# arkworks-rs/marlin

Measured on NVIDIA H100. Metric: prover_constraints_per_sec, higher is better.
Workload: dtype u32-limb modular integers (Fr 255-bit, Fq 381-bit)

## Files before the change

marlin_b200/csrc/msm.cuh:

```cuda
#pragma once
#include "common.cuh"
#include "curve.cuh"
#include "msm_layout.hpp"

namespace b2m {

constexpr uint32_t MSM_BKT_MASK = (1u << MSM_BKT_BITS) - 1;
constexpr uint32_t MSM_NO_DIGIT = 0xffffffffu;
constexpr int MSM_MAX_AFFINE_LEVELS = 6;

template <class Fr, class Fq>
struct MsmJob {
  const Fr* scalars;
  bool mont;
  size_t n;
  size_t base_off;
  const Fr* scalars2;
  size_t n2;
  size_t extra_base;
  const XYZZ<Fq>* extra;
  int n_extra;
  XYZZ<Fq>* out_xyzz;
  Affine<Fq>* out_affine;
  size_t scalar_stride = 1;
};

template <class Fr, class Fq>
struct Msm {
  Ctx* ctx;
  size_t n_srs = 0;
  size_t n_srs_global = 0;
  int tab_rank = 0, tab_world = 1;
  size_t n_extra = 0;
  size_t stride = 0;
  int c = 0, W = 0;
  int T = 0, m = 1;
  size_t max_pairs = 0;
  int affine_levels = Fq::N > 8 ? 3 : 0;
  int affine_ctas_upper = 22;
  int affine_ctas = 4;
  size_t affine_min_refs = MSM_AFFINE_MIN_REFS;
  int affine_map = 1;
  int affine_T = 64;
  int affine_T_upper = 32;
  int acc_ctas_per_sm = 3;
  DBuf<Affine<Fq>> tables;

  static int pick_window(size_t n);
  Msm(Ctx& cx, const Affine<Fq>* powers, size_t n, const Affine<Fq>* host_extra, size_t n_extra_bases, int window_bits,
      bool powers_on_device = false, int n_tables = 0, size_t max_pairs = 0);

  void run(const Fr* scalars, bool mont, size_t n, size_t base_off, const XYZZ<Fq>* extra, int n_extra, XYZZ<Fq>* out_xyzz,
           Affine<Fq>* out_affine);
  void run_batch(const MsmJob<Fr, Fq>* jobs, int nj);
  void run_pass(const MsmJob<Fr, Fq>* jobs, int nj);
  void run_host(size_t base_off, const uint64_t* scalars, size_t n, uint64_t* out_xy, int* out_is_inf);
  void read_power(size_t i, uint64_t* out_xy);
  static void g1_to_bytes(Ctx& cx, const Affine<Fq>* dev_pts, const uint64_t* host_pts, size_t n, uint8_t* out);
  static void g1_from_bytes(Ctx& cx, const uint8_t* bytes, size_t n, uint64_t* out_xy);
  static void g1_powers_host(Ctx& cx, const uint64_t* g_xy, const uint64_t* beta, size_t n, uint64_t* out);
  static void fixed_base_host(Ctx& cx, const uint64_t* g_xy, const uint64_t* scalars, const uint64_t* beta, size_t first, size_t n, uint64_t* out);
};

}
```

marlin_b200/csrc/msm_affine.cuh:

```cuda
#pragma once
#include "curve.cuh"
#ifdef __CUDACC__
#include "devmem.cuh"
#else
struct uint2 {
  uint32_t x, y;
};
struct uint4 {
  uint32_t x, y, z, w;
};
#endif

namespace b2m {

constexpr uint32_t AFF_BKT_BITS = 24;

template <class Fq>
struct AffLevel {
  const Affine<Fq>* tables;
  size_t table_stride;
  const uint2* sorted;
  const Affine<Fq>* in;
  const uint32_t* off_in;
  const uint32_t* off_out;
  uint32_t B;
  Affine<Fq>* out;
  uint2* out_refs;
  Fq* pref;
  uint4* meta;
  uint32_t T, nthreads;
  uint32_t lane_step;
  Fq* inv;
};

struct AffMap {
  uint32_t o0, step, cnt;
};
template <class Fq>
B2M_HD AffMap aff_map(const AffLevel<Fq>& A, uint32_t t, uint32_t total) {
  AffMap m;
  m.step = A.lane_step;
  uint64_t o0;
  if (A.lane_step == 1) {
    o0 = (uint64_t)t * A.T;
  } else {
    o0 = (uint64_t)(t / A.lane_step) * A.lane_step * A.T + (t % A.lane_step);
  }
  if (o0 >= total) {
    m.o0 = 0;
    m.cnt = 0;
    return m;
  }
  m.o0 = (uint32_t)o0;
  const uint32_t left = (total - m.o0 + m.step - 1) / m.step;
  m.cnt = left < A.T ? left : A.T;
  return m;
}

#if defined(__CUDA_ARCH__)
#define B2M_AFF_LDG(p) ldg_words(p)
#define B2M_AFF_LD(p) ld_words(p)
#define B2M_AFF_ST(p, v) st_words(p, v)
#define B2M_AFF_LDG32(p) __ldg(p)
#else
#define B2M_AFF_LDG(p) (*(p))
#define B2M_AFF_LD(p) (*(p))
#define B2M_AFF_ST(p, v) (*(p) = (v))
#define B2M_AFF_LDG32(p) (*(p))
#endif

B2M_HD uint32_t aff_bucket_of(const uint32_t* off, uint32_t n, uint32_t v) {
  uint32_t lo = 0, hi = n;
  while (hi - lo > 1) {
    uint32_t mid = (lo + hi) >> 1;
    if (B2M_AFF_LDG32(off + mid) <= v) lo = mid; else hi = mid;
  }
  return lo;
}

template <class Fq, bool L0>
B2M_HD void aff_plan_thread(const AffLevel<Fq>& A, uint32_t t) {
  const uint32_t total = B2M_AFF_LDG32(A.off_out + A.B);
  const AffMap mp = aff_map(A, t, total);
  if (!mp.cnt) return;
  uint32_t b = aff_bucket_of(A.off_out, A.B, mp.o0);
  uint32_t b_start = B2M_AFF_LDG32(A.off_out + b), b_end = B2M_AFF_LDG32(A.off_out + b + 1);
  for (uint32_t k = 0; k < mp.cnt; k++) {
    const uint32_t o = mp.o0 + k * mp.step;
    if (o >= b_end) {
      int steps = 0;
      do {
        b++;
        b_end = B2M_AFF_LDG32(A.off_out + b + 1);
      } while (o >= b_end && ++steps < 8);
      if (o >= b_end) {
        b = aff_bucket_of(A.off_out, A.B, o);
        b_end = B2M_AFF_LDG32(A.off_out + b + 1);
      }
      b_start = B2M_AFF_LDG32(A.off_out + b);
    }
    const uint32_t in_start = B2M_AFF_LDG32(A.off_in + b), in_end = B2M_AFF_LDG32(A.off_in + b + 1);
    const uint32_t i0 = in_start + 2u * (o - b_start);
    const bool pair = i0 + 1u < in_end;
    uint4 m;
    if (L0) {
      const uint2 r0 = B2M_AFF_LDG32(A.sorted + i0);
      m.x = (uint32_t)((size_t)(r0.y >> AFF_BKT_BITS) * A.table_stride + (r0.x & 0x7fffffffu)) | (r0.x & 0x80000000u);
      m.y = m.x;
      if (pair) {
        const uint2 r1 = B2M_AFF_LDG32(A.sorted + i0 + 1u);
        m.y = (uint32_t)((size_t)(r1.y >> AFF_BKT_BITS) * A.table_stride + (r1.x & 0x7fffffffu)) | (r1.x & 0x80000000u);
      }
    } else {
      m.x = i0;
      m.y = pair ? i0 + 1u : i0;
    }
    m.z = b;
    m.w = pair ? 1u : 0u;
    A.meta[(size_t)k * A.nthreads + t] = m;
  }
}

template <class Fq>
B2M_HD Fq aff_ldx(const Affine<Fq>* base, uint32_t ref) {
  return B2M_AFF_LDG(&base[ref & 0x7fffffffu].x);
}
template <class Fq>
B2M_HD Affine<Fq> aff_ld(const Affine<Fq>* base, uint32_t ref) {
  const Affine<Fq>* p = base + (ref & 0x7fffffffu);
  Affine<Fq> r;
  r.x = B2M_AFF_LDG(&p->x);
  r.y = B2M_AFF_LDG(&p->y);
  return r;
}
template <class Fq>
B2M_HD Affine<Fq> aff_signed(Affine<Fq> p, uint32_t ref) {
  if (ref >> 31) p.y = p.y.neg();
  return p;
}

enum AffKind : uint32_t { AFF_COPY_P = 0, AFF_COPY_Q = 1, AFF_INF = 2, AFF_ADD = 3, AFF_DBL = 4 };

template <class Fq>
B2M_HD AffKind aff_classify(const Affine<Fq>& P, const Affine<Fq>& Q, Fq* den) {
  if (P.is_inf()) return AFF_COPY_Q;
  if (Q.is_inf()) return AFF_COPY_P;
  if (P.x == Q.x) {
    if (P.y == Q.y && !P.y.is_zero()) {
      *den = P.y.dbl();
      return AFF_DBL;
    }
    return AFF_INF;
  }
  *den = Q.x - P.x;
  return AFF_ADD;
}

template <class Fq, bool PF>
B2M_HD void aff_level_thread(const AffLevel<Fq>& A, const Affine<Fq>* base, uint32_t t) {
  const uint32_t total = B2M_AFF_LDG32(A.off_out + A.B);
// ... 280 lines not shown
```

marlin_b200/csrc/msm_impl.cuh:

```cuda
#pragma once
#include "msm.cuh"
#include "devmem.cuh"
#include "scan.cuh"
#include "msm_affine.cuh"
#include "comm.cuh"

namespace b2m {

template <class Fq>
__device__ __forceinline__ Affine<Fq> ld_affine(const Affine<Fq>* p) {
  Affine<Fq> r;
  const uint4* q = reinterpret_cast<const uint4*>(p);
  uint32_t* d = reinterpret_cast<uint32_t*>(&r);
#pragma unroll
  for (int i = 0; i < 2 * Fq::N / 4; i++) {
    uint4 v = __ldg(q + i);
    d[4 * i] = v.x; d[4 * i + 1] = v.y; d[4 * i + 2] = v.z; d[4 * i + 3] = v.w;
  }
  return r;
}
template <class Fq> __device__ __noinline__ void g1_add(XYZZ<Fq>& a, const XYZZ<Fq>& b) { a.add(b); }
template <class Fq> __device__ __noinline__ void g1_add_mixed(XYZZ<Fq>& a, const Affine<Fq>& b) { a.add_mixed(b); }
template <class Fq> __device__ __noinline__ void g1_dbl(XYZZ<Fq>& a) { a = a.dbl(); }
template <class Fq> __device__ __noinline__ Fq fq_inverse(const Fq& a) { return a.inverse_fast(); }
// ... 67 lines not shown
      carry = 0;
      out = v ? (set_off + v - 1) : MSM_NO_DIGIT;
    }
    digits[(size_t)w * nt + i] = out;
    if (out != MSM_NO_DIGIT) atomicAdd(hist + (out & 0x7fffffffu), 1u);
  }
}


static __global__ void msm_scatter_kernel(const uint32_t* digits, size_t n, size_t nt, size_t base_off, size_t idx2, int W, int m,
                                          uint32_t* cursor, uint2* sorted) {
  size_t i = blockIdx.x * (size_t)blockDim.x + threadIdx.x;
  if (i >= nt) return;
  uint32_t abs_idx = (uint32_t)(i < n ? base_off + i : idx2 + (i - n));
  for (int w = 0; w < W; w++) {
    uint32_t d = digits[(size_t)w * nt + i];
    if (d == MSM_NO_DIGIT) continue;
    uint32_t bkt = d & 0x7fffffffu;
    uint32_t pos = atomicAdd(cursor + bkt, 1u);
    sorted[pos] = make_uint2(abs_idx | (d & 0x80000000u), bkt | ((uint32_t)(w / m) << MSM_BKT_BITS));
  }
}

constexpr int MSM_Q = 64;
constexpr int MSM_Q_MIN = 32;
template <class Fq>
__global__ void __launch_bounds__(128)
msm_accumulate_kernel(const Affine<Fq>* __restrict__ tables, size_t table_stride, const uint32_t* __restrict__ offsets,
                      const uint32_t* __restrict__ ends, const uint2* __restrict__ sorted, const uint32_t* __restrict__ total_refs_p,
                      const uint32_t q, XYZZ<Fq>* __restrict__ buckets, XYZZ<Fq>* __restrict__ part_pt,
                      uint32_t* __restrict__ part_bkt) {
  const uint32_t total = *total_refs_p;
  const uint32_t t = blockIdx.x * blockDim.x + threadIdx.x;
  const uint64_t start64 = (uint64_t)t * q;
  uint32_t head_b = MSM_NO_DIGIT, tail_b = MSM_NO_DIGIT;
  if (start64 < total) {
    const uint32_t start = (uint32_t)start64;
    const uint32_t end = (total - start > q) ? start + q : total;
    uint2 rb = __ldg(sorted + start);
    uint32_t ref = rb.x;
    uint32_t cur_b = rb.y & MSM_BKT_MASK;
    uint32_t seg_start = start;
    Affine<Fq> p = ld_affine(tables + (size_t)(rb.y >> MSM_BKT_BITS) * table_stride + (ref & 0x7fffffffu));
    XYZZ<Fq> acc = XYZZ<Fq>::inf();
    for (uint32_t e = start; e < end; e++) {
      Affine<Fq> cur = p;
      const bool neg = ref >> 31;
      uint32_t next_b = cur_b;
      if (e + 1 < end) {
        rb = __ldg(sorted + e + 1);
        ref = rb.x;
        next_b = rb.y & MSM_BKT_MASK;
        p = ld_affine(tables + (size_t)(rb.y >> MSM_BKT_BITS) * table_stride + (ref & 0x7fffffffu));
      }
      acc.add_mixed(cur, neg);
      if (e + 1 == end || next_b != cur_b) {
        const bool whole = (seg_start == offsets[cur_b]) && (e + 1 == ends[cur_b]);
        if (whole) {
          st_words(buckets + cur_b, acc);
        } else if (seg_start == start && head_b == MSM_NO_DIGIT) {
          st_words(part_pt + 2 * (size_t)t, acc);
          head_b = cur_b;
        } else {
          st_words(part_pt + 2 * (size_t)t + 1, acc);
          tail_b = cur_b;
        }
        acc = XYZZ<Fq>::inf();
        seg_start = e + 1;
        cur_b = next_b;
      }
    }
  }
  part_bkt[2 * (size_t)t] = head_b;
  part_bkt[2 * (size_t)t + 1] = tail_b;
}
static __global__ void msm_level_counts_kernel(const uint32_t* off_in, uint32_t B, uint32_t* cnt) {
  uint32_t b = blockIdx.x * blockDim.x + threadIdx.x;
  if (b > B) return;
  cnt[b] = b < B ? (off_in[b + 1] - off_in[b] + 1u) / 2u : 0u;
}
template <class Fq, bool L0>
__global__ void __launch_bounds__(256) msm_affine_plan_kernel(const AffLevel<Fq> A) {
  const uint32_t t = blockIdx.x * blockDim.x + threadIdx.x;
  if (t < A.nthreads) aff_plan_thread<Fq, L0>(A, t);
}
template <class Fq, int MINB, bool PF>
__global__ void __launch_bounds__(128, MINB) msm_affine_level_kernel(const AffLevel<Fq> A, const Affine<Fq>* __restrict__ base) {
  const uint32_t t = blockIdx.x * blockDim.x + threadIdx.x;
  if (t < A.nthreads) aff_level_thread<Fq, PF>(A, base, t);
}

template <class Fq, int MINB, int PHASE, bool PIPE = true>
__global__ void __launch_bounds__(128, MINB) msm_affine_level_sp_kernel(const AffLevel<Fq> A, const Affine<Fq>* __restrict__ base) {
  const uint32_t t = blockIdx.x * blockDim.x + threadIdx.x;
  if (t < A.nthreads) aff_level_thread_sp<Fq, PHASE, PIPE>(A, base, t);
}

template <class Fq>
__device__ __forceinline__ Fq shfl_fq(const Fq& a, int src_lane) {
  Fq r;
#pragma unroll
  for (int i = 0; i < Fq::N; i++) r.l[i] = __shfl_sync(0xffffffffu, a.l[i], src_lane);
  return r;
}
template <class Fq>
__global__ void __launch_bounds__(128) fq_batch_inverse_kernel(Fq* v, size_t n) {
  constexpr int G = 4;
  const size_t t = blockIdx.x * (size_t)blockDim.x + threadIdx.x;
  const int lane = threadIdx.x & 31;
  const size_t i0 = t * G;
  Fq e[G], pre[G];
  Fq run = Fq::one();
#pragma unroll
  for (int k = 0; k < G; k++) {
    e[k] = i0 + k < n ? ld_words(v + i0 + k) : Fq::one();
    pre[k] = run;
    run = run * e[k];
  }
  Fq pin = run, sin = run;
#pragma unroll
  for (int d = 1; d < 32; d <<= 1) {
    const Fq up = shfl_fq(pin, lane - d < 0 ? lane : lane - d);
    const Fq dn = shfl_fq(sin, lane + d > 31 ? lane : lane + d);
    if (lane >= d) pin = pin * up;
    if (lane + d <= 31) sin = sin * dn;
  }
  Fq tinv = Fq::one();
  if (lane == 31) tinv = fq_inverse(pin);
  tinv = shfl_fq(tinv, 31);
  Fq before = shfl_fq(pin, lane == 0 ? 0 : lane - 1), after = shfl_fq(sin, lane == 31 ? 31 : lane + 1);
  if (lane == 0) before = Fq::one();
  if (lane == 31) after = Fq::one();
  Fq inv_run = tinv * before * after;
#pragma unroll
  for (int k = G - 1; k >= 0; k--) {
    const Fq ek = inv_run * pre[k];
    inv_run = inv_run * e[k];
    if (i0 + k < n) st_words(v + i0 + k, ek);
  }
}

struct MsmLongRun {
  uint32_t first, last, bucket;
  uint32_t dst;
};
constexpr uint32_t MSM_RUN_CHUNK = 256;
constexpr uint32_t MSM_RUN_SHORT = 12;
template <class Fq>
__global__ void __launch_bounds__(128)
msm_stitch_kernel(const XYZZ<Fq>* part_pt, const uint32_t* part_bkt, size_t nthreads, const uint32_t q, const uint32_t* offsets,
                  const uint32_t* ends, XYZZ<Fq>* buckets, MsmLongRun* long_runs, MsmLongRun* final_runs, MsmLongRun* short_runs, uint32_t* n_long,
                  uint32_t long_cap, uint32_t chunk_cap) {
  size_t u = blockIdx.x * (size_t)blockDim.x + threadIdx.x;
  if (u >= nthreads) return;
  uint32_t first = 2u * (uint32_t)u + 1u;
  uint32_t b = part_bkt[first];
  if (b == MSM_NO_DIGIT) {
    first = 2u * (uint32_t)u;
    b = part_bkt[first];
    if (b == MSM_NO_DIGIT || offsets[b] != (uint32_t)u * q) return;
  }
  const uint32_t t1 = (ends[b] - 1u) / q;
  const uint32_t last = 2u * t1;
  if (t1 > (uint32_t)u + 1u) {
    const uint32_t nslots = last - first + 1u;
    if (nslots <= MSM_RUN_SHORT) {
      const uint32_t slot = atomicAdd(n_long + 3, 1u);
      if (slot < long_cap) {
        short_runs[slot] = MsmLongRun{first, last, b, MSM_NO_DIGIT};
        return;
      }
    } else if (nslots <= MSM_RUN_CHUNK) {
      const uint32_t slot = atomicAdd(n_long, 1u);
      if (slot < long_cap) {
        long_runs[slot] = MsmLongRun{first, last, b, MSM_NO_DIGIT};
        return;
      }
    } else {
// ... 310 lines not shown
    const bool inf = (p.y.l[Fq::N - 1] >> 30) & 1u;
    p.y.l[Fq::N - 1] &= 0x3fffffffu;
    p.x = Fq::from_canonical(p.x);
    p.y = Fq::from_canonical(p.y);
    if (inf) p = Affine<Fq>::inf();
  }
  st_words(out + i, p);
}

template <class Fr, class Fq>
int Msm<Fr, Fq>::pick_window(size_t n) {
  int lg = 0;
  while (((size_t)1 << (lg + 1)) <= n) lg++;
  int c = lg >= 21 ? 20 : (lg >= 17 ? 16 : lg - 1);
  if (c < MSM_MIN_WINDOW) c = MSM_MIN_WINDOW;
  if (c > 20) c = 20;
  auto top_bits = [](int w) {
    const int W = (Fr::Params::BITS + 1 + w - 1) / w;
    return Fr::Params::BITS + 1 - (W - 1) * w;
  };
  if (top_bits(c) < 6) {
    if (c + 1 <= 20 && top_bits(c + 1) >= 6) c = c + 1;
    else if (c - 1 >= MSM_MIN_WINDOW && top_bits(c - 1) >= 6) c = c - 1;
    else if (c - 2 >= MSM_MIN_WINDOW && top_bits(c - 2) >= 6) c = c - 2;
  }
  return c;
}

template <class Fr, class Fq>
Msm<Fr, Fq>::Msm(Ctx& cx, const Affine<Fq>* host_powers, size_t n, const Affine<Fq>* host_extra, size_t n_extra_bases, int window_bits,
                 bool powers_on_device, int n_tables, size_t max_pairs_)
    : ctx(&cx), n_extra(n_extra_bases), n_srs_global(n), max_pairs(max_pairs_) {
  B2M_REQUIRE(!powers_on_device || cx.world <= 1, B2M_ERR_UNSUPPORTED, "device-resident bases on a multi-GPU context");
  tab_world = cx.world > 1 ? cx.world : 1;
  tab_rank = cx.world > 1 ? cx.rank : 0;
  n_srs = n > (size_t)tab_rank ? (n - tab_rank + tab_world - 1) / tab_world : 0;
  stride = n_srs + n_extra;
  B2M_REQUIRE(n >= 1 && stride < ((size_t)1 << 31), B2M_ERR_INVALID_ARG, "SRS size %zu out of range", n);
  c = window_bits > 0 ? window_bits : pick_window(n / (size_t)tab_world);
  B2M_REQUIRE(c >= MSM_MIN_WINDOW && c <= 24, B2M_ERR_INVALID_ARG, "window bits %d out of range [%d, 24]", c, MSM_MIN_WINDOW);
  W = (Fr::Params::BITS + 1 + c - 1) / c;
  B2M_REQUIRE(W <= 32, B2M_ERR_INVALID_ARG, "too many windows (%d)", W);
  T = n_tables > 0 && n_tables < W ? msm_tables_used(W, n_tables) : W;
  B2M_REQUIRE((T == W && max_pairs == 0) || tab_world == 1, B2M_ERR_UNSUPPORTED,
              "reduced window tables (%d of %d) or an MSM pass cap (%zu pairs) on a multi-GPU context", T, W, max_pairs);
  m = msm_sets(W, T);
  B2M_REQUIRE(msm_sets_fit(c, m), B2M_ERR_INVALID_ARG, "%d window tables at c = %d: %d bucket sets of 2^%d buckets exceed the 2^%d bucket ids", T, c,
              m, c - 1, MSM_BKT_BITS);
  tables = DBuf<Affine<Fq>>(cx, (size_t)T * stride);
  if (powers_on_device) {
    B2M_CUDA(cudaMemcpyAsync(tables.p, host_powers, n * sizeof(Affine<Fq>), cudaMemcpyDeviceToDevice, cx.stream));
  } else if (tab_world == 1) {
    tables.upload(host_powers, n);
  } else if (n_srs) {
    DBuf<Affine<Fq>> all(cx, n);
    all.upload(host_powers, n);
    msm_take_residue_kernel<Fq><<<div_up(n_srs, 256), 256, 0, cx.stream>>>(all.p, n_srs, tab_rank, tab_world, tables.p);
    B2M_CHECK_LAUNCH();
    cx.launches++;
  }
  if (n_extra) B2M_CUDA(cudaMemcpyAsync(tables.p + n_srs, host_extra, n_extra * sizeof(Affine<Fq>), cudaMemcpyHostToDevice, cx.stream));
  if (stride) {
    msm_precompute_kernel<Fq><<<div_up(stride, 128), 128, 0, cx.stream>>>(tables.p, stride, c * m, T);
    B2M_CHECK_LAUNCH();
    cx.launches++;
  }
  cx.sync();
  B2M_CUDA(cudaOccupancyMaxActiveBlocksPerMultiprocessor(&acc_ctas_per_sm, msm_accumulate_kernel<Fq>, 128, 0));
  if (acc_ctas_per_sm < 1) acc_ctas_per_sm = 1;
  if (const char* e = getenv("B2M_MSM_AFFINE_LEVELS")) affine_levels = atoi(e);
  if (const char* e = getenv("B2M_MSM_AFFINE_T")) affine_T = affine_T_upper = atoi(e);
  if (const char* e = getenv("B2M_MSM_AFFINE_T_UPPER")) affine_T_upper = atoi(e);
  if (const char* e = getenv("B2M_MSM_AFFINE_CTAS")) affine_ctas = atoi(e);
  if (const char* e = getenv("B2M_MSM_AFFINE_CTAS_UPPER")) affine_ctas_upper = atoi(e);
  if (const char* e = getenv("B2M_MSM_AFFINE_MIN_REFS")) affine_min_refs = (size_t)atoll(e);
  if (const char* e = getenv("B2M_MSM_AFFINE_MAP")) affine_map = atoi(e);

  if (affine_levels < 0) affine_levels = 0;
  if (affine_levels > MSM_MAX_AFFINE_LEVELS) affine_levels = MSM_MAX_AFFINE_LEVELS;
  if (affine_T < 1) affine_T = 1;
  if (affine_T > 1024) affine_T = 1024;
  if (affine_T_upper < 1) affine_T_upper = 1;
  if (affine_T_upper > 1024) affine_T_upper = 1024;
}

template <class Fr, class Fq>
void Msm<Fr, Fq>::run(const Fr* scalars, bool mont, size_t n, size_t base_off, const XYZZ<Fq>* extra, int n_extra,
                      XYZZ<Fq>* out_xyzz, Affine<Fq>* out_affine) {
  MsmJob<Fr, Fq> job{scalars, mont, n, base_off, nullptr, 0, 0, extra, n_extra, out_xyzz, out_affine};
  run_batch(&job, 1);
}

template <class Fr, class Fq>
void Msm<Fr, Fq>::run_batch(const MsmJob<Fr, Fq>* jobs, int nj) {
  B2M_REQUIRE(nj >= 1 && nj <= MSM_MAX_BATCH, B2M_ERR_INVALID_ARG, "MSM batch of %d jobs", nj);
  size_t passes = 1;
  for (int j = 0; j < nj && max_pairs; j++) passes = std::max(passes, (jobs[j].n + max_pairs - 1) / max_pairs);
  if (passes == 1) {
    run_pass(jobs, nj);
    return;
  }
  Ctx& cx = *ctx;
  for (int j = 0; j < nj; j++)
    B2M_REQUIRE(jobs[j].base_off + jobs[j].n <= n_srs_global, B2M_ERR_DEGREE_TOO_LARGE, "MSM slice [%zu, %zu) exceeds the SRS (%zu powers)",
                jobs[j].base_off, jobs[j].base_off + jobs[j].n, n_srs_global);
  DBuf<XYZZ<Fq>> partial(cx, passes * nj);
  partial.zero();
  for (size_t p = 0; p < passes; p++) {
    MsmJob<Fr, Fq> sub[MSM_MAX_BATCH];
    int ns = 0;
    const size_t at = p * max_pairs;
    for (int j = 0; j < nj; j++) {
      if (p > 0 && at >= jobs[j].n) continue;
      MsmJob<Fr, Fq> s = jobs[j];
      s.n = at < jobs[j].n ? std::min(max_pairs, jobs[j].n - at) : 0;
      s.scalars = jobs[j].scalars + at * jobs[j].scalar_stride;
      s.base_off = jobs[j].base_off + at;
      if (p > 0) { s.scalars2 = nullptr; s.n2 = 0; }
      s.extra = nullptr; s.n_extra = 0;
      s.out_xyzz = partial.p + p * nj + j; s.out_affine = nullptr;
      sub[ns++] = s;
    }
    run_pass(sub, ns);
  }
  MsmFinishJobs fj;
  for (int j = 0; j < nj; j++) fj.j[j] = MsmFinishJob{jobs[j].extra, jobs[j].n_extra, jobs[j].out_xyzz, jobs[j].out_affine};
  msm_combine_kernel<Fq><<<nj, 32, 0, cx.stream>>>(partial.p, (int)passes, nj, fj);
  B2M_CHECK_LAUNCH();
  cx.launches++;
}

template <class Fr, class Fq>
void Msm<Fr, Fq>::run_pass(const MsmJob<Fr, Fq>* jobs_in, int nj) {
  Ctx& cx = *ctx;
  B2M_REQUIRE(nj >= 1 && nj <= MSM_MAX_BATCH, B2M_ERR_INVALID_ARG, "MSM batch of %d jobs", nj);
  MsmJob<Fr, Fq> local[MSM_MAX_BATCH];
  const bool sharded = cx.world > 1;
  B2M_REQUIRE((sharded ? cx.world : 1) == tab_world && (sharded ? cx.rank : 0) == tab_rank, B2M_ERR_INVALID_ARG,
              "this key's tables were built for rank %d of %d; create the SRS after b2m_ctx_attach_comm", tab_rank, tab_world);
  DBuf<XYZZ<Fq>> partial, gathered;
  if (sharded) {
    partial = DBuf<XYZZ<Fq>>(cx, nj);
    gathered = DBuf<XYZZ<Fq>>(cx, (size_t)nj * cx.world);
  }
  for (int j = 0; j < nj; j++) {
    local[j] = jobs_in[j];
    B2M_REQUIRE(jobs_in[j].base_off + jobs_in[j].n <= n_srs_global, B2M_ERR_DEGREE_TOO_LARGE,
                "MSM slice [%zu, %zu) exceeds the SRS (%zu powers)", jobs_in[j].base_off, jobs_in[j].base_off + jobs_in[j].n, n_srs_global);
    if (sharded) {
      const size_t G = (size_t)cx.world, off = jobs_in[j].base_off, n = jobs_in[j].n;
      const size_t skip = ((size_t)cx.rank + G - off % G) % G;
      const size_t cnt = n > skip ? (n - skip + G - 1) / G : 0;
      local[j].scalars = jobs_in[j].scalars + skip;
      local[j].scalar_stride = G;
      local[j].base_off = (off + skip) / G;
      local[j].n = cnt;
      if (cx.rank != 0) { local[j].scalars2 = nullptr; local[j].n2 = 0; }
      local[j].extra = nullptr; local[j].n_extra = 0;
      local[j].out_xyzz = partial.p + j; local[j].out_affine = nullptr;
    }
  }
  const MsmJob<Fr, Fq>* jobs = local;
  size_t max_n = 0;
  for (int j = 0; j < nj; j++) {
    B2M_REQUIRE(jobs[j].n == 0 || jobs[j].base_off + jobs[j].n <= n_srs, B2M_ERR_DEGREE_TOO_LARGE, "MSM slot range [%zu, %zu) exceeds the tables (%zu)",
                jobs[j].base_off, jobs[j].base_off + jobs[j].n, n_srs);
    B2M_REQUIRE(jobs[j].n2 == 0 || jobs[j].extra_base + jobs[j].n2 <= n_extra, B2M_ERR_INVALID_ARG, "extra bases out of range");
    max_n = std::max(max_n, jobs[j].n + jobs[j].n2);
  }
  B2M_REQUIRE((size_t)W * max_n < ((size_t)1 << 32), B2M_ERR_DEGREE_TOO_LARGE, "MSM of %zu pairs x %d windows exceeds 2^32 bucket references", max_n, W);
  MsmFinishJobs fj;
  for (int j = 0; j < nj; j++) fj.j[j] = MsmFinishJob{jobs[j].extra, jobs[j].n_extra, jobs[j].out_xyzz, jobs[j].out_affine};
  auto exchange = [&]() {
    if (!sharded) return;
    size_t spx = cx.span_begin("msm_allgather", (double)nj);
    all_gather_bytes(cx, partial.p, gathered.p, (size_t)nj * sizeof(XYZZ<Fq>));
    MsmFinishJobs oj;
    for (int j = 0; j < nj; j++) oj.j[j] = MsmFinishJob{jobs_in[j].extra, jobs_in[j].n_extra, jobs_in[j].out_xyzz, jobs_in[j].out_affine};
    msm_combine_kernel<Fq><<<nj, 32, 0, cx.stream>>>(gathered.p, cx.world, nj, oj);
    B2M_CHECK_LAUNCH();
    cx.launches++;
    cx.span_end(spx);
  };
  if (max_n == 0) {
    msm_finish_kernel<Fq><<<nj, 64, 0, cx.stream>>>(nullptr, 0, nullptr, 0, 0, fj);
    B2M_CHECK_LAUNCH();
    cx.launches++;
    exchange();
    return;
  }
  const uint32_t B = 1u << (c - 1);
  const uint32_t NB = (uint32_t)m * B;
  const size_t G = (size_t)nj * m;
  const int cbits = (c - 1 + 1) / 2, rbits = (c - 1) - cbits;
  const size_t L = (size_t)1 << cbits, R = (size_t)1 << rbits;
  DBuf<XYZZ<Fq>> buckets(cx, (size_t)nj * NB);
  {
    const size_t max_refs = (size_t)W * max_n;
    const int LV = max_refs >= affine_min_refs ? affine_levels : 0;
    size_t bound[MSM_MAX_AFFINE_LEVELS + 1];
    bound[0] = max_refs;
    for (int l = 1; l <= LV; l++) bound[l] = (bound[l - 1] + NB) / 2 + 1;
    size_t lvl_cap[2] = {0, 0};
    for (int l = 0; l < LV; l++) lvl_cap[l & 1] = std::max(lvl_cap[l & 1], bound[l + 1]);
    const size_t acc_refs = LV > 0 ? std::max(max_refs, bound[LV]) : max_refs;
    const size_t max_threads = (acc_refs + MSM_Q_MIN - 1) / MSM_Q_MIN + 256;
    DBuf<uint32_t> digits[2], hist[2], offsets[2], cursor[2];
    DBuf<uint2> sorted[2];
    const int slots = nj > 1 ? 2 : 1;
    for (int s = 0; s < slots; s++) {
      digits[s] = DBuf<uint32_t>(cx, max_refs); hist[s] = DBuf<uint32_t>(cx, NB + 1); offsets[s] = DBuf<uint32_t>(cx, NB + 1);
      cursor[s] = DBuf<uint32_t>(cx, NB); sorted[s] = DBuf<uint2>(cx, max_refs);
    }
    DBuf<uint32_t> part_bkt(cx, 2 * max_threads), n_long(cx, 4);
    const uint32_t long_cap = 1u << 18;
    const uint32_t chunk_cap = (uint32_t)(4 * max_threads / MSM_RUN_CHUNK + 4);
    DBuf<MsmLongRun> long_runs(cx, long_cap), short_runs(cx, long_cap), final_runs(cx, chunk_cap);
    DBuf<XYZZ<Fq>> chunk_pt(cx, chunk_cap);
    DBuf<XYZZ<Fq>> part_pt(cx, 2 * max_threads);
    B2M_REQUIRE(LV == 0 || (size_t)T * stride < ((size_t)1 << 31), B2M_ERR_DEGREE_TOO_LARGE,
                "window tables of %d x %zu entries exceed the 31-bit index of the batched-affine plan", T, stride);
    DBuf<Affine<Fq>> lvl_pts[2];
    DBuf<uint32_t> lvl_off[2], lvl_cnt;
    DBuf<uint2> lvl_refs;
    DBuf<uint4> lvl_meta;
    DBuf<Fq> lvl_pref, lvl_inv;
    if (LV > 0) {
      lvl_pts[0] = DBuf<Affine<Fq>>(cx, lvl_cap[0]);
      if (LV > 1) lvl_pts[1] = DBuf<Affine<Fq>>(cx, lvl_cap[1]);
      lvl_off[0] = DBuf<uint32_t>(cx, NB + 1); lvl_off[1] = DBuf<uint32_t>(cx, NB + 1); lvl_cnt = DBuf<uint32_t>(cx, NB + 1);
      lvl_refs = DBuf<uint2>(cx, bound[LV]);
      const size_t T_max = (size_t)std::max(affine_T, affine_T_upper), T_min = (size_t)std::min(affine_T, affine_T_upper);
      const size_t slots_l0 = T_max * ((std::max(lvl_cap[0], lvl_cap[1]) + T_max - 1) / T_max + 128);
      lvl_meta = DBuf<uint4>(cx, slots_l0);
      lvl_pref = DBuf<Fq>(cx, slots_l0);
      lvl_inv = DBuf<Fq>(cx, slots_l0 / T_min + 256);
    }
    buckets.zero();
    cudaEvent_t ev_ready, ev_sorted[MSM_MAX_BATCH], ev_acc[MSM_MAX_BATCH];
    B2M_CUDA(cudaEventCreateWithFlags(&ev_ready, cudaEventDisableTiming));
    for (int j = 0; j < nj; j++) {
      B2M_CUDA(cudaEventCreateWithFlags(&ev_sorted[j], cudaEventDisableTiming));
      B2M_CUDA(cudaEventCreateWithFlags(&ev_acc[j], cudaEventDisableTiming));
    }
    B2M_CUDA(cudaEventRecord(ev_ready, cx.stream));
    B2M_CUDA(cudaStreamWaitEvent(cx.side, ev_ready, 0));
    for (int j = 0; j < nj; j++) {
      const size_t n = jobs[j].n, nt = jobs[j].n + jobs[j].n2;
      const int s = j % slots;
      if (nt == 0) {
        B2M_CUDA(cudaEventRecord(ev_acc[j], cx.stream));
        continue;
      }
      {
        StreamSwap on_side(cx, cx.side);
        if (j >= slots) B2M_CUDA(cudaStreamWaitEvent(cx.side, ev_acc[j - slots], 0));
        hist[s].zero();
        size_t sp0 = cx.span_begin("msm_sort", (double)n);
        msm_digits_kernel<Fr><<<div_up(nt, 256), 256, 0, cx.stream>>>(jobs[j].scalars, jobs[j].scalar_stride, jobs[j].scalars2, jobs[j].mont, n, nt, c, W,
                                                                      m, digits[s].p, hist[s].p);
        B2M_CHECK_LAUNCH();
        exclusive_scan_u32(cx, hist[s].p, offsets[s].p, NB + 1);
        B2M_CUDA(cudaMemcpyAsync(cursor[s].p, offsets[s].p, NB * sizeof(uint32_t), cudaMemcpyDeviceToDevice, cx.stream));
        msm_scatter_kernel<<<div_up(nt, 256), 256, 0, cx.stream>>>(digits[s].p, n, nt, jobs[j].base_off, n_srs + jobs[j].extra_base, W, m,
                                                                    cursor[s].p, sorted[s].p);
        B2M_CHECK_LAUNCH();
        cx.launches += 2;
        cx.span_end(sp0);
        B2M_CUDA(cudaEventRecord(ev_sorted[j], cx.side));
      }
      B2M_CUDA(cudaStreamWaitEvent(cx.stream, ev_sorted[j], 0));
      const Affine<Fq>* src_tables = tables.p;
      size_t src_stride = stride;
      const uint32_t* src_off = offsets[s].p;
      const uint2* src_sorted = sorted[s].p;
      size_t refs = (size_t)W * nt;
      if (LV > 0 && refs >= affine_min_refs) {
        size_t spl = cx.span_begin("msm_affine_levels", (double)n);
        bound[0] = refs;
        for (int l = 1; l <= LV; l++) bound[l] = (bound[l - 1] + NB) / 2 + 1;
        const uint32_t* off_in = offsets[s].p;
        for (int l = 0; l < LV; l++) {
          uint32_t* off_out = lvl_off[l & 1].p;
          msm_level_counts_kernel<<<div_up((size_t)NB + 1, 256), 256, 0, cx.stream>>>(off_in, NB, lvl_cnt.p);
          B2M_CHECK_LAUNCH();
          cx.launches++;
          exclusive_scan_u32(cx, lvl_cnt.p, off_out, (size_t)NB + 1);
          const uint32_t lane_step = affine_map ? 32u : 1u;
          const size_t T_l = (size_t)(l == 0 ? affine_T : affine_T_upper);
          const uint32_t nthreads = (uint32_t)(lane_step * ((bound[l + 1] + (size_t)lane_step * T_l - 1) / ((size_t)lane_step * T_l)));
          AffLevel<Fq> A{tables.p, stride, sorted[s].p, l > 0 ? lvl_pts[(l - 1) & 1].p : nullptr, off_in, off_out, NB, lvl_pts[l & 1].p,
                         l == LV - 1 ? lvl_refs.p : nullptr, lvl_pref.p, lvl_meta.p, (uint32_t)T_l, nthreads, lane_step, lvl_inv.p};
          if (l == 0)
            msm_affine_plan_kernel<Fq, true><<<div_up(nthreads, 256), 256, 0, cx.stream>>>(A);
          else
            msm_affine_plan_kernel<Fq, false><<<div_up(nthreads, 256), 256, 0, cx.stream>>>(A);
          const Affine<Fq>* base = l == 0 ? tables.p : lvl_pts[(l - 1) & 1].p;
          const unsigned grid = div_up(nthreads, 128);
          const int variant = l == 0 ? affine_ctas : affine_ctas_upper;
          static const char* const lvl_names[MSM_MAX_AFFINE_LEVELS] = {"msm_aff_level0", "msm_aff_level1", "msm_aff_level2", "msm_aff_level3",
                                                                       "msm_aff_level4", "msm_aff_level5"};
          const size_t spk = cx.span_begin(lvl_names[l], (double)n);
          switch (variant) {
            case 3: msm_affine_level_kernel<Fq, 3, true><<<grid, 128, 0, cx.stream>>>(A, base); break;
            case 5: msm_affine_level_kernel<Fq, 5, false><<<grid, 128, 0, cx.stream>>>(A, base); break;
            case 8: msm_affine_level_sp_kernel<Fq, 3, 0><<<grid, 128, 0, cx.stream>>>(A, base); break;
            case 9: msm_affine_level_sp_kernel<Fq, 2, 0><<<grid, 128, 0, cx.stream>>>(A, base); break;
            case 11: case 12: case 13:
              msm_affine_level_sp_kernel<Fq, 5, 1><<<grid, 128, 0, cx.stream>>>(A, base);
              if (variant == 11) msm_affine_level_sp_kernel<Fq, 3, 2><<<grid, 128, 0, cx.stream>>>(A, base);
              else if (variant == 12) msm_affine_level_sp_kernel<Fq, 2, 2><<<grid, 128, 0, cx.stream>>>(A, base);
              else msm_affine_level_sp_kernel<Fq, 4, 2, false><<<grid, 128, 0, cx.stream>>>(A, base);
              cx.launches++;
              break;
            case 21: case 22:
              msm_affine_level_sp_kernel<Fq, 6, 3><<<grid, 128, 0, cx.stream>>>(A, base);
              fq_batch_inverse_kernel<Fq><<<div_up(div_up(nthreads, 4), 128), 128, 0, cx.stream>>>(lvl_inv.p, nthreads);
              if (variant == 21) msm_affine_level_sp_kernel<Fq, 4, 2, false><<<grid, 128, 0, cx.stream>>>(A, base);
              else msm_affine_level_sp_kernel<Fq, 3, 2><<<grid, 128, 0, cx.stream>>>(A, base);
              cx.launches += 2;
              break;
            default: msm_affine_level_kernel<Fq, 4, false><<<grid, 128, 0, cx.stream>>>(A, base); break;
          }
          cx.span_end(spk);
          B2M_CHECK_LAUNCH();
          cx.launches += 2;
          off_in = off_out;
        }
        cx.span_end(spl);
        src_tables = lvl_pts[(LV - 1) & 1].p;
        src_stride = 0;
        src_off = off_in;
        src_sorted = lvl_refs.p;
        refs = bound[LV];
      }
      const uint32_t* src_ends = src_off + 1;
      const uint32_t* src_total = src_off + NB;
      size_t sp = cx.span_begin("msm_accumulate_kernel", (double)n);
      const size_t wave = (size_t)cx.sm_count * acc_ctas_per_sm * 128;
      size_t waves = (refs + wave * MSM_Q / 2) / (wave * MSM_Q);
      if (waves < 1) waves = 1;
      uint32_t q = (uint32_t)((refs + waves * wave - 1) / (waves * wave));
      if (q < (uint32_t)MSM_Q_MIN) q = MSM_Q_MIN;
      const size_t nthreads = (refs + q - 1) / q;
      msm_accumulate_kernel<Fq><<<div_up(nthreads, 128), 128, 0, cx.stream>>>(src_tables, src_stride, src_off, src_ends, src_sorted,
                                                                               src_total, q, buckets.p + (size_t)j * NB, part_pt.p,
                                                                               part_bkt.p);
      B2M_CHECK_LAUNCH();
      cx.launches++;
      cx.span_end(sp);
      size_t sp1 = cx.span_begin("msm_stitch", (double)n);
      n_long.zero();
      msm_stitch_kernel<Fq><<<div_up(nthreads, 128), 128, 0, cx.stream>>>(part_pt.p, part_bkt.p, nthreads, q, src_off, src_ends,
                                                                           buckets.p + (size_t)j * NB, long_runs.p, final_runs.p, short_runs.p, n_long.p,
                                                                           long_cap, chunk_cap);
      msm_stitch_short_kernel<Fq><<<2 * cx.sm_count, 128, 0, cx.stream>>>(part_pt.p, part_bkt.p, short_runs.p, n_long.p + 3, long_cap,
                                                                          buckets.p + (size_t)j * NB);
      msm_stitch_runs_kernel<Fq, false><<<4 * cx.sm_count, 128, 0, cx.stream>>>(part_pt.p, part_bkt.p, long_runs.p, n_long.p, long_cap,
                                                                                buckets.p + (size_t)j * NB, chunk_pt.p);
      msm_stitch_runs_kernel<Fq, true><<<cx.sm_count, 128, 0, cx.stream>>>(part_pt.p, part_bkt.p, final_runs.p, n_long.p + 1, chunk_cap,
                                                                           buckets.p + (size_t)j * NB, chunk_pt.p);
      B2M_CHECK_LAUNCH();
      cx.launches += 4;
      cx.span_end(sp1);
      B2M_CUDA(cudaEventRecord(ev_acc[j], cx.stream));
    }
    cudaEventDestroy(ev_ready);
    for (int j = 0; j < nj; j++) {
      cudaEventDestroy(ev_sorted[j]);
      cudaEventDestroy(ev_acc[j]);
    }
  }
  double units = 0;
  for (int j = 0; j < nj; j++) units += (double)jobs[j].n;
  size_t sp2 = cx.span_begin("msm_reduce", units);
  DBuf<XYZZ<Fq>> rsum(cx, G * R), csum(cx, G * L);
  {
    const uint32_t Kr = (uint32_t)std::min<size_t>(L, 8), Kc = (uint32_t)std::min<size_t>(R, 8);
    const size_t seg_r = L / Kr, seg_c = R / Kc;
    DBuf<XYZZ<Fq>> part_r(cx, G * R * seg_r), part_c(cx, G * L * seg_c);
    msm_segsum_kernel<Fq><<<div_up(G * R * seg_r, 128), 128, 0, cx.stream>>>(buckets.p, part_r.p, G, seg_r, Kr, R, 1, L, B);
    msm_segsum_kernel<Fq><<<div_up(G * L * seg_c, 128), 128, 0, cx.stream>>>(buckets.p, part_c.p, G, seg_c, Kc, L, L, 1, B);
    const MsmFoldJob fr{part_r.p, rsum.p, G * R, seg_r}, fc{part_c.p, csum.p, G * L, seg_c};
    msm_fold_kernel<Fq><<<div_up((G * R + G * L) * 32, 128), 128, 0, cx.stream>>>(fr, fc);
    B2M_CHECK_LAUNCH();
    cx.launches += 3;
  }
  DBuf<XYZZ<Fq>> rplanes(cx, G * (rbits + 1)), cplanes(cx, G * (cbits + 1));
  msm_bitplane_kernel<Fq><<<dim3(rbits + 1 + cbits + 1, (unsigned)G), 256, 0, cx.stream>>>(rsum.p, R, rbits, rplanes.p, csum.p, L, cbits, cplanes.p);
  B2M_CHECK_LAUNCH();
  cx.launches++;
  if (m == 1) {
    msm_finish_kernel<Fq><<<nj, 64, 0, cx.stream>>>(rplanes.p, rbits, cplanes.p, cbits, 1, fj);
    B2M_CHECK_LAUNCH();
    cx.launches++;
  } else {
    DBuf<XYZZ<Fq>> set_sums(cx, G);
    msm_set_sum_kernel<Fq><<<(unsigned)G, 64, 0, cx.stream>>>(rplanes.p, rbits, cplanes.p, cbits, set_sums.p);
    msm_sets_finish_kernel<Fq><<<nj, 32, 0, cx.stream>>>(set_sums.p, m, c, fj);
    B2M_CHECK_LAUNCH();
    cx.launches += 2;
  }
  cx.span_end(sp2);
  exchange();
// ... 91 lines not shown
```

Measured before the change: 4.116 million.

## Stream upper-level affine operands into shared memory via bulk async copies

Adds a new level-kernel variant (23), now the default for upper affine levels. It precomputes per-warp-step contiguous input ranges in the plan kernel, then uses cp.async.bulk with mbarriers to stream each warp's 64-point operand window into shared memory through a multi-stage pipeline. Both the denominator/prefix pass and the backward add pass read operands from shared memory instead of scattered global loads. The aim is to hide global memory latency for affine point fetches, at the cost of extra planning work, dynamic shared memory that may reduce occupancy, and use of bulk-copy PTX (cp.async.bulk, mbarrier expect_tx) that needs sm_90 or later.

After: 4.235 million (median of 6 runs). 1.03x the previous value.

```diff
diff --git a/marlin_b200/csrc/msm.cuh b/marlin_b200/csrc/msm.cuh
--- a/marlin_b200/csrc/msm.cuh
+++ b/marlin_b200/csrc/msm.cuh
@@ -37,7 +37,7 @@
   int T = 0, m = 1;
   size_t max_pairs = 0;
   int affine_levels = Fq::N > 8 ? 3 : 0;
-  int affine_ctas_upper = 22;
+  int affine_ctas_upper = 23;
   int affine_ctas = 4;
   size_t affine_min_refs = MSM_AFFINE_MIN_REFS;
   int affine_map = 1;
diff --git a/marlin_b200/csrc/msm_affine.cuh b/marlin_b200/csrc/msm_affine.cuh
--- a/marlin_b200/csrc/msm_affine.cuh
+++ b/marlin_b200/csrc/msm_affine.cuh
@@ -31,6 +31,7 @@
   uint32_t T, nthreads;
   uint32_t lane_step;
   Fq* inv;
+  uint2* rng;
 };
 
 struct AffMap {
@@ -76,6 +77,35 @@
     if (B2M_AFF_LDG32(off + mid) <= v) lo = mid; else hi = mid;
   }
   return lo;
+}
+
+constexpr uint32_t AFF_STEP_PTS = 64;
+B2M_HD uint2 aff_step_range(const uint32_t* off_in, const uint32_t* off_out, uint32_t B, uint32_t T, uint32_t w, uint32_t k) {
+  uint2 r;
+  r.x = 0;
+  r.y = 0;
+  const uint32_t total = B2M_AFF_LDG32(off_out + B);
+  const uint64_t oa = ((uint64_t)w * T + k) * 32u;
+  if (k >= T || oa >= total) return r;
+  const uint32_t o_a = (uint32_t)oa, o_b = total - o_a > 32u ? o_a + 31u : total - 1u;
+  const uint32_t ba = aff_bucket_of(off_out, B, o_a);
+  uint32_t lo = ba, hi = B;
+  while (hi - lo > 1) {
+    const uint32_t mid = (lo + hi) >> 1;
+    if (B2M_AFF_LDG32(off_out + mid) <= o_b) lo = mid; else hi = mid;
+  }
+  const uint32_t bb = lo;
+  const uint32_t first = B2M_AFF_LDG32(off_in + ba) + 2u * (o_a - B2M_AFF_LDG32(off_out + ba));
+  const uint32_t i_b = B2M_AFF_LDG32(off_in + bb) + 2u * (o_b - B2M_AFF_LDG32(off_out + bb));
+  const uint32_t end_b = B2M_AFF_LDG32(off_in + bb + 1);
+  r.x = first;
+  r.y = (i_b + 2u < end_b ? i_b + 2u : end_b) - first;
+  return r;
+}
+template <class Fq>
+B2M_HD void aff_plan_ranges_thread(const AffLevel<Fq>& A, uint32_t t) {
+  const uint32_t w = t / 32u;
+  for (uint32_t k = t % 32u; k < A.T; k += 32u) A.rng[(size_t)w * A.T + k] = aff_step_range(A.off_in, A.off_out, A.B, A.T, w, k);
 }
 
 template <class Fq, bool L0>
diff --git a/marlin_b200/csrc/msm_impl.cuh b/marlin_b200/csrc/msm_impl.cuh
--- a/marlin_b200/csrc/msm_impl.cuh
+++ b/marlin_b200/csrc/msm_impl.cuh
@@ -173,7 +173,10 @@
 template <class Fq, bool L0>
 __global__ void __launch_bounds__(256) msm_affine_plan_kernel(const AffLevel<Fq> A) {
   const uint32_t t = blockIdx.x * blockDim.x + threadIdx.x;
-  if (t < A.nthreads) aff_plan_thread<Fq, L0>(A, t);
+  if (t < A.nthreads) {
+    aff_plan_thread<Fq, L0>(A, t);
+    if (A.rng) aff_plan_ranges_thread<Fq>(A, t);
+  }
 }
 template <class Fq, int MINB, bool PF>
 __global__ void __launch_bounds__(128, MINB) msm_affine_level_kernel(const AffLevel<Fq> A, const Affine<Fq>* __restrict__ base) {
@@ -185,6 +188,159 @@
 __global__ void __launch_bounds__(128, MINB) msm_affine_level_sp_kernel(const AffLevel<Fq> A, const Affine<Fq>* __restrict__ base) {
   const uint32_t t = blockIdx.x * blockDim.x + threadIdx.x;
   if (t < A.nthreads) aff_level_thread_sp<Fq, PHASE, PIPE>(A, base, t);
+}
+
+extern __shared__ __align__(128) unsigned char aff_stream_smem[];
+
+template <class Fq, int S>
+struct AffStream {
+  static constexpr uint32_t STAGE = AFF_STEP_PTS * sizeof(Affine<Fq>);
+  static constexpr size_t smem_bytes(int warps) { return (size_t)warps * S * STAGE; }
+  const Affine<Fq>* in;
+  const uint2* rng;
+  uint32_t nsteps, lane, wi;
+  uint32_t bar_s;
+  uint2 chunk_r;
+  int chunk;
+  __device__ __forceinline__ void init(const AffLevel<Fq>& A, const Affine<Fq>* base, uint64_t* bars, uint32_t t, uint32_t n) {
+    in = base;
+    lane = t & 31u;
+    wi = threadIdx.x >> 5;
+    rng = A.rng + (size_t)(t >> 5) * A.T;
+    nsteps = n;
+    chunk = -1;
+    bar_s = (uint32_t)__cvta_generic_to_shared(bars + wi * S);
+    if (lane == 0) {
+      for (int s = 0; s < S; s++) asm volatile("mbarrier.init.shared::cta.b64 [%0], 1;" ::"r"(bar_s + 8u * s));
+      asm volatile("fence.mbarrier_init.release.cluster;" ::: "memory");
+    }
+    __syncwarp();
+  }
+  __device__ __forceinline__ const Affine<Fq>* stage(uint32_t s) const {
+    return reinterpret_cast<const Affine<Fq>*>(aff_stream_smem + (wi * S + s) * STAGE);
+  }
+  __device__ __forceinline__ void issue(uint32_t k, uint32_t s) {
+    if ((int)(k >> 5) != chunk) {
+      chunk = (int)(k >> 5);
+      const uint32_t j = (k & ~31u) + lane;
+      chunk_r = j < nsteps ? __ldg(rng + j) : make_uint2(0u, 0u);
+    }
+    const uint32_t lo = __shfl_sync(0xffffffffu, chunk_r.x, k & 31u), n = __shfl_sync(0xffffffffu, chunk_r.y, k & 31u);
+    if (lane == 0) {
+      const uint32_t bar = bar_s + 8u * s, bytes = n * (uint32_t)sizeof(Affine<Fq>);
+      const uint32_t dst = (uint32_t)__cvta_generic_to_shared(stage(s));
+      asm volatile("fence.proxy.async.shared::cta;" ::: "memory");
+      asm volatile("mbarrier.arrive.expect_tx.shared::cta.b64 _, [%0], %1;" ::"r"(bar), "r"(bytes) : "memory");
+      asm volatile("cp.async.bulk.shared::cluster.global.mbarrier::complete_tx::bytes [%0], [%1], %2, [%3];" ::"r"(dst), "l"(in + lo),
+                   "r"(bytes), "r"(bar)
+                   : "memory");
+    }
+  }
+  __device__ __forceinline__ void wait(uint32_t s, uint32_t parity) const {
+    uint32_t done = 0;
+    while (!done) {
+      asm volatile("{\n .reg .pred p;\n mbarrier.try_wait.parity.shared::cta.b64 p, [%1], %2;\n selp.u32 %0, 1, 0, p;\n}"
+                   : "=r"(done)
+                   : "r"(bar_s + 8u * s), "r"(parity)
+                   : "memory");
+    }
+  }
+};
+
+template <class Fq, int MINB, int S>
+__global__ void __launch_bounds__(128, MINB) msm_affine_stream_den_kernel(const AffLevel<Fq> A, const Affine<Fq>* __restrict__ base) {
+  __shared__ __align__(8) uint64_t bars[4 * S];
+  const uint32_t t = blockIdx.x * blockDim.x + threadIdx.x;
+  if (t >= A.nthreads) return;
+  const uint32_t total = __ldg(A.off_out + A.B);
+  const AffMap mp = aff_map(A, t, total);
+  const uint32_t cnt = mp.cnt;
+  const uint32_t nsteps = __shfl_sync(0xffffffffu, cnt, 0);
+  Fq run = Fq::one();
+  if (nsteps) {
+    AffStream<Fq, S> R;
+    R.init(A, base, bars, t, nsteps);
+    const size_t nth = A.nthreads;
+    const uint4* meta = A.meta + t;
+    Fq* pref = A.pref + t;
+    for (uint32_t s = 0; s < (uint32_t)S && s < nsteps; s++) R.issue(s, s);
+    uint4 m = cnt ? meta[0] : make_uint4(0u, 0u, 0u, 0u);
+    uint4 m1 = cnt > 1 ? meta[nth] : m;
+    for (uint32_t k = 0; k < nsteps; k++) {
+      const uint32_t s = k % S;
+      const uint4 mc = m;
+      const uint32_t lo = __shfl_sync(0xffffffffu, mc.x, 0);
+      R.wait(s, (k / S) & 1u);
+      Fq c1, c2;
+      if (k < cnt) {
+        c1 = ld_words(&R.stage(s)[mc.x - lo].x);
+        c2 = ld_words(&R.stage(s)[mc.y - lo].x);
+      }
+      __syncwarp();
+      if (k + S < nsteps) R.issue(k + S, s);
+      if (k + 1 < cnt) {
+        m = m1;
+        if (k + 2 < cnt) m1 = meta[(size_t)(k + 2) * nth];
+      }
+      if (k < cnt) {
+        const Fq d = c2 - c1;
+        const Fq den = aff_fast(mc.w, c1, c2) ? d : Fq::one();
+        st_words(pref + (size_t)k * nth, run);
+        run = run * den;
+      }
+    }
+  }
+  st_words(A.inv + t, run);
+}
+
+template <class Fq, int MINB, int S>
+__global__ void __launch_bounds__(128, MINB) msm_affine_stream_add_kernel(const AffLevel<Fq> A, const Affine<Fq>* __restrict__ base) {
+  __shared__ __align__(8) uint64_t bars[4 * S];
+  const uint32_t t = blockIdx.x * blockDim.x + threadIdx.x;
+  if (t >= A.nthreads) return;
+  const uint32_t total = __ldg(A.off_out + A.B);
+  const AffMap mp = aff_map(A, t, total);
+  const uint32_t cnt = mp.cnt;
+  const uint32_t nsteps = __shfl_sync(0xffffffffu, cnt, 0);
+  if (!nsteps) return;
+  AffStream<Fq, S> R;
+  R.init(A, base, bars, t, nsteps);
+  const size_t nth = A.nthreads;
+  const uint4* meta = A.meta + t;
+  const Fq* pref = A.pref + t;
+  Fq inv = ld_words(A.inv + t);
+  const uint32_t K = nsteps - 1;
+  for (uint32_t i = 0; i < (uint32_t)S && i < nsteps; i++) R.issue(K - i, i);
+  uint4 m = K < cnt ? meta[(size_t)K * nth] : make_uint4(0u, 0u, 0u, 0u);
+  for (uint32_t i = 0; i < nsteps; i++) {
+    const uint32_t k = K - i, s = i % S;
+    const bool act = k < cnt;
+    const uint4 mc = m;
+    if (k > 0) m = meta[(size_t)(k - 1) * nth];
+    const Fq pf = act ? ld_words(pref + (size_t)k * nth) : Fq::one();
+    const uint32_t lo = __shfl_sync(0xffffffffu, mc.x, 0);
+    R.wait(s, (i / S) & 1u);
+    Affine<Fq> P, Q;
+    if (act) {
+      P = ld_words(R.stage(s) + (mc.x - lo));
+      Q = ld_words(R.stage(s) + (mc.y - lo));
+    }
+    __syncwarp();
+    if (i + S < nsteps) R.issue(k - S, s);
+    if (act) {
+      const bool fast = aff_fast(mc.w, P.x, Q.x);
+      const Fq d = Q.x - P.x;
+      const Fq den = fast ? d : Fq::one();
+      const Fq dinv = inv * pf;
+      inv = inv * den;
+      const Fq lam = (Q.y - P.y) * dinv;
+      Affine<Fq> Rp;
+      Rp.x = lam.sqr() - P.x - Q.x;
+      Rp.y = lam * (P.x - Rp.x) - P.y;
+      if (!fast) Rp = aff_add_slow(P, Q, mc.w);
+      aff_store_out(A, mp.o0 + k * mp.step, Rp, mc.z);
+    }
+  }
 }
 
 template <class Fq>
@@ -661,6 +817,7 @@
   if (affine_T > 1024) affine_T = 1024;
   if (affine_T_upper < 1) affine_T_upper = 1;
   if (affine_T_upper > 1024) affine_T_upper = 1024;
+  B2M_REQUIRE(affine_ctas != 23, B2M_ERR_INVALID_ARG, "level-kernel variant 23 streams contiguous operands: levels >= 1 only (B2M_MSM_AFFINE_CTAS_UPPER)");
 }
 
 template <class Fr, class Fq>
@@ -804,6 +961,8 @@
     DBuf<uint2> lvl_refs;
     DBuf<uint4> lvl_meta;
     DBuf<Fq> lvl_pref, lvl_inv;
+    DBuf<uint2> lvl_rng;
+    const int variant_upper = affine_ctas_upper == 23 && !affine_map ? 22 : affine_ctas_upper;
     if (LV > 0) {
       lvl_pts[0] = DBuf<Affine<Fq>>(cx, lvl_cap[0]);
       if (LV > 1) lvl_pts[1] = DBuf<Affine<Fq>>(cx, lvl_cap[1]);
@@ -814,6 +973,7 @@
       lvl_meta = DBuf<uint4>(cx, slots_l0);
       lvl_pref = DBuf<Fq>(cx, slots_l0);
       lvl_inv = DBuf<Fq>(cx, slots_l0 / T_min + 256);
+      if (LV > 1 && variant_upper == 23) lvl_rng = DBuf<uint2>(cx, slots_l0 / 32 + 32);
     }
     buckets.zero();
     cudaEvent_t ev_ready, ev_sorted[MSM_MAX_BATCH], ev_acc[MSM_MAX_BATCH];
@@ -868,15 +1028,16 @@
           const uint32_t lane_step = affine_map ? 32u : 1u;
           const size_t T_l = (size_t)(l == 0 ? affine_T : affine_T_upper);
           const uint32_t nthreads = (uint32_t)(lane_step * ((bound[l + 1] + (size_t)lane_step * T_l - 1) / ((size_t)lane_step * T_l)));
+          const int variant = l == 0 ? affine_ctas : variant_upper;
           AffLevel<Fq> A{tables.p, stride, sorted[s].p, l > 0 ? lvl_pts[(l - 1) & 1].p : nullptr, off_in, off_out, NB, lvl_pts[l & 1].p,
-                         l == LV - 1 ? lvl_refs.p : nullptr, lvl_pref.p, lvl_meta.p, (uint32_t)T_l, nthreads, lane_step, lvl_inv.p};
+                         l == LV - 1 ? lvl_refs.p : nullptr, lvl_pref.p, lvl_meta.p, (uint32_t)T_l, nthreads, lane_step, lvl_inv.p,
+                         variant == 23 ? lvl_rng.p : nullptr};
           if (l == 0)
             msm_affine_plan_kernel<Fq, true><<<div_up(nthreads, 256), 256, 0, cx.stream>>>(A);
           else
             msm_affine_plan_kernel<Fq, false><<<div_up(nthreads, 256), 256, 0, cx.stream>>>(A);
           const Affine<Fq>* base = l == 0 ? tables.p : lvl_pts[(l - 1) & 1].p;
           const unsigned grid = div_up(nthreads, 128);
-          const int variant = l == 0 ? affine_ctas : affine_ctas_upper;
           static const char* const lvl_names[MSM_MAX_AFFINE_LEVELS] = {"msm_aff_level0", "msm_aff_level1", "msm_aff_level2", "msm_aff_level3",
                                                                        "msm_aff_level4", "msm_aff_level5"};
           const size_t spk = cx.span_begin(lvl_names[l], (double)n);
@@ -899,6 +1060,17 @@
               else msm_affine_level_sp_kernel<Fq, 3, 2><<<grid, 128, 0, cx.stream>>>(A, base);
               cx.launches += 2;
               break;
+            case 23: {
+              constexpr int S_DEN = 2, S_ADD = 3;
+              const size_t sm_den = AffStream<Fq, S_DEN>::smem_bytes(4), sm_add = AffStream<Fq, S_ADD>::smem_bytes(4);
+              B2M_CUDA(cudaFuncSetAttribute(msm_affine_stream_den_kernel<Fq, 4, S_DEN>, cudaFuncAttributeMaxDynamicSharedMemorySize, (int)sm_den));
+              B2M_CUDA(cudaFuncSetAttribute(msm_affine_stream_add_kernel<Fq, 3, S_ADD>, cudaFuncAttributeMaxDynamicSharedMemorySize, (int)sm_add));
+              msm_affine_stream_den_kernel<Fq, 4, S_DEN><<<grid, 128, sm_den, cx.stream>>>(A, base);
+              fq_batch_inverse_kernel<Fq><<<div_up(div_up(nthreads, 4), 128), 128, 0, cx.stream>>>(lvl_inv.p, nthreads);
+              msm_affine_stream_add_kernel<Fq, 3, S_ADD><<<grid, 128, sm_add, cx.stream>>>(A, base);
+              cx.launches += 2;
+              break;
+            }
             default: msm_affine_level_kernel<Fq, 4, false><<<grid, 128, 0, cx.stream>>>(A, base); break;
           }
           cx.span_end(spk);
```
